# zc402/video-classification

Hardware: AMD Instinct MI355X
Metric: clips/sec SlowFast-R50 8x8, 32x224^2 bf16 training step (higher is better)
Workload: dtype bf16

## Files before the change

### video-classification_amd/csrc/conv_igemm.hip

```cpp

#include "conv_igemm_epi.h"

using namespace sfk_igemm;

namespace sfk_igemm {
__attribute__((visibility("hidden"))) int launch_p8(const ConvK& k, int bms, dim3 grid, hipStream_t s, int* dry);
__attribute__((visibility("hidden"))) bool halo_ok(const sfk_conv_desc* d);
__attribute__((visibility("hidden"))) int halo_mtiles(const sfk_conv_desc* d);
__attribute__((visibility("hidden"))) int launch_halo(const ConvK& k, const sfk_conv_desc* d, hipStream_t s, int* dry);
}

namespace {

template <typename T, int BM, int BN, int WM, int WN, bool SHORTK, int EPI = 0>
__global__ __launch_bounds__(256, (sizeof(T) == 2 ? 3 : 1)) void conv_igemm_kernel(const ConvK k) {
  using TL = Tile<T>;
  constexpr int VEC = TL::VEC, SEGS = TL::SEGS, ROWB = TL::ROWB;
  constexpr int FM = BM / WM / 16, FN = co_frags(BN, WN);
  constexpr int RPI = 256 / SEGS;
  constexpr int XL = BM / RPI;
  constexpr int WL = (BN + RPI - 1) / RPI;
  constexpr int BUF = (BM + BN) * ROWB;
  static_assert(WM * WN == 4 && BM % RPI == 0, "tile shape");
  __shared__ __attribute__((aligned(16))) char smem[2 * BUF];
  __shared__ sfk_tap s_taps[SFK_MAX_TAPS + 1];
  __shared__ int s_xdelta[SFK_MAX_TAPS + 1];
  __shared__ int s_woff[SFK_MAX_TAPS + 1];
  if (threadIdx.x <= SFK_MAX_TAPS) {
    sfk_tap t = k.taps[threadIdx.x < SFK_MAX_TAPS ? threadIdx.x : 0];
    if ((int)threadIdx.x >= k.ntaps) { t.dt = -128; t.dh = 0; t.dw = 0; t.widx = 0; }
    s_taps[threadIdx.x] = t;
    s_xdelta[threadIdx.x] = (((int)t.dt * k.xh + (int)t.dh) * k.xw + (int)t.dw) * k.xld * (int)sizeof(T);
    s_woff[threadIdx.x] = (int)t.widx * k.cin * (int)sizeof(T);
  }
  __syncthreads();

  const int tid = threadIdx.x, lane = tid & 63, wave = tid >> 6;
  const int wm = wave % WM, wn = wave / WM;
  const int l15 = lane & 15, g = lane >> 4;

  int mt, nt;
  {
    const int nblk = gridDim.x, b = blockIdx.x;
    const int q = nblk >> 3, r = nblk & 7, xcd = b & 7;
    const int logical = (xcd < r ? xcd * (q + 1) : r * (q + 1) + (xcd - r) * q) + (b >> 3);
    nt = logical % k.ntiles;
    mt = logical / k.ntiles;
  }

  const int seg = tid % SEGS, row0 = tid / SEGS;
  int xtb[XL], xhb[XL], xwb[XL];
  uint32_t xbase[XL];
#pragma unroll
  for (int i = 0; i < XL; ++i) {
    const int m = mt * BM + row0 + i * RPI;
    uint32_t q1, rw_, q2, rh_, n_, rt_;
    k.drw.divmod((uint32_t)m, q1, rw_);
    k.drh.divmod(q1, q2, rh_);
    k.drt.divmod(q2, n_, rt_);
    xtb[i] = (m < k.M) ? (int)rt_ * k.gst : -(1 << 28);
    xhb[i] = (int)rh_ * k.gsh;
    xwb[i] = (int)rw_ * k.gsw;
    xbase[i] = (uint32_t)((((((int64_t)n_ * k.xt + (int)rt_ * k.gst) * k.xh + xhb[i]) * k.xw + xwb[i]) * k.xld + k.xoff) *
                          (int64_t)sizeof(T));
  }
  uint32_t wbase[WL];
#pragma unroll
  for (int i = 0; i < WL; ++i) {
    const int r = row0 + i * RPI;
    const int co = nt * BN + r;
    wbase[i] = (r < BN && co < k.cout) ? (uint32_t)(co * k.wtaps * k.cin) * (uint32_t)sizeof(T) : SFK_OOB;
  }
  const __amdgpu_buffer_rsrc_t xrs = sfk_make_rsrc(k.x, k.xbytes);
  const __amdgpu_buffer_rsrc_t wrs = sfk_make_rsrc(k.w, k.wbytes);

  struct Stage { uint4 x[XL]; uint4 w[WL]; };
  auto gload = [&](int step, Stage& st) {
    const uint32_t q = (uint32_t)(step * SEGS + seg);
    uint32_t tap, cseg;
    k.dspt.divmod(q, tap, cseg);
    const bool cok = tap < (uint32_t)k.ntaps;
    const int ti_ = cok ? (int)tap : SFK_MAX_TAPS;
    const sfk_tap tp = s_taps[ti_];
    const uint32_t xd = (uint32_t)(s_xdelta[ti_] + (int)cseg * 16);
    const uint32_t wd = (uint32_t)(s_woff[ti_] + (int)cseg * 16);
#pragma unroll
    for (int i = 0; i < XL; ++i) {
      const int ti = xtb[i] + tp.dt, hi = xhb[i] + tp.dh, wi = xwb[i] + tp.dw;
      const bool ok = cok && (unsigned)ti < (unsigned)k.xt && (unsigned)hi < (unsigned)k.xh &&
                      (unsigned)wi < (unsigned)k.xw;
      st.x[i] = sfk_buffer_load16(xrs, ok ? xbase[i] + xd : SFK_OOB);
    }
#pragma unroll
    for (int i = 0; i < WL; ++i)
      st.w[i] = sfk_buffer_load16(wrs, (cok && wbase[i] != SFK_OOB) ? wbase[i] + wd : SFK_OOB);
  };
  auto lstore = [&](int buf, const Stage& st) {
    char* xs = smem + buf * BUF;
    char* ws = xs + BM * ROWB;
#pragma unroll
    for (int i = 0; i < XL; ++i) *reinterpret_cast<uint4*>(xs + TL::off(row0 + i * RPI, seg)) = st.x[i];
#pragma unroll
    for (int i = 0; i < WL; ++i) {
      const int r = row0 + i * RPI;
      if ((BN % RPI == 0) || r < BN) *reinterpret_cast<uint4*>(ws + TL::off(r, seg)) = st.w[i];
    }
  };

  f32x4 acc[FN][FM];
#pragma unroll
  for (int i = 0; i < FN; ++i)
#pragma unroll
    for (int j = 0; j < FM; ++j) acc[i][j] = f32x4{0.f, 0.f, 0.f, 0.f};

  auto compute = [&](int buf) {
    const char* xs = smem + buf * BUF;
    const char* ws = xs + BM * ROWB;
    typename TL::frag a[FN], b[FM];
#pragma unroll
    for (int i = 0; i < FN; ++i) a[i] = TL::load(ws, wn * (BN / WN) + 16 * i + l15, g);
#pragma unroll
    for (int j = 0; j < FM; ++j) b[j] = TL::load(xs, wm * (BM / WM) + 16 * j + l15, g);
#pragma unroll
    for (int i = 0; i < FN; ++i)
#pragma unroll
      for (int j = 0; j < FM; ++j) TL::mma(acc[i][j], a[i], b[j]);
  };

  Stage r0, r1;
  if constexpr (SHORTK) {
    gload(0, r0);
    lstore(0, r0);
    if (k.KC > 1) gload(1, r1);
    __syncthreads();
    int it = 0;
    for (; it + 3 < k.KC; it += 2) {
      gload(it + 2, r0);
      compute(0);
      lstore(1, r1);
      __syncthreads();
      gload(it + 3, r1);
      compute(1);
      lstore(0, r0);
      __syncthreads();
    }
    const int rem = k.KC - it;
    if (rem == 1) {
      compute(0);
    } else if (rem == 2) {
      compute(0);
      lstore(1, r1);
      __syncthreads();
      compute(1);
    } else {
      gload(it + 2, r0);
      compute(0);
      lstore(1, r1);
      __syncthreads();
      compute(1);
      lstore(0, r0);
      __syncthreads();
      compute(0);
    }
  } else {
    const int nit2 = (k.KC + 1) & ~1;
    gload(0, r0);
    lstore(0, r0);
    gload(1, r1);
    __syncthreads();
    for (int it = 0; it < nit2; it += 2) {
      gload(it + 2, r0);
      compute(0);
      lstore(1, r1);
      __syncthreads();
      gload(it + 3, r1);
      compute(1);
      lstore(0, r0);
      __syncthreads();
    }
  }

  if constexpr ((EPI == 1 || EPI >= 5) && sizeof(T) == 2 && (FN % 2) == 0) {
    __syncthreads();
    if constexpr (EPI == 5) epilogue_bits_sum<FM, FN, BM, BN, WM, WN>(k, acc, reinterpret_cast<float*>(smem), mt, nt, wm, wn, lane, tid);
    else epilogue_bn_bwd<FM, FN, BM, BN, WM, WN, EPI == 6, EPI == 7>(k, acc, reinterpret_cast<float*>(smem), mt, nt, wm, wn, lane, tid);
    return;
  }
  if constexpr (EPI == 3) {
    epilogue_fused<T, FM, FN, BM, BN, WM, WN>(k, acc, mt, nt, wm, wn, lane);
    return;
  }
  epilogue_plain<T, EPI, FM, FN, BM, BN, WM, WN, true>(k, acc, reinterpret_cast<float*>(smem), mt, nt, wm, wn, lane, tid);
}

typedef __attribute__((address_space(3))) void lds_void_t;

template <int BM, int BN, int WM, int WN, int EPI = 0, int BMS = BM>
__global__ __launch_bounds__(64 * WM * WN, (BN == 256 ? 2 : (WM * WN == 8 ? 4 : 3))) void conv_igemm_dma_kernel(const ConvK k) {
  using T = bf16_t;
  using TL = Tile<bf16_t>;
  constexpr int VEC = 8, SEGS = 4, ROWB = 64;
  constexpr int FM = BMS / WM / 16, FN = co_frags(BN, WN);
  static_assert(BMS <= BM && BMS % (16 * WM) == 0, "computed rows");
  constexpr int NW = WM * WN;
  constexpr int WROWS = BN < 16 * NW ? 16 * NW : BN;
  constexpr int XI = BM / (16 * NW), WI = WROWS / (16 * NW);
  constexpr int BUF = (BM + WROWS) * ROWB;
  constexpr int RED = WM * BN * 2 * 4;
  constexpr int SM = 3 * BUF > RED ? 3 * BUF : RED;
  constexpr int TAB = 32;
  static_assert((NW == 4 || NW == 8) && BM % (16 * NW) == 0, "tile shape");
  __shared__ __attribute__((aligned(16))) char smem[SM + 3 * TAB * 4];
  sfk_tap* s_taps = reinterpret_cast<sfk_tap*>(smem + SM);
  int* s_xdelta = reinterpret_cast<int*>(smem + SM) + TAB;
  int* s_woff = reinterpret_cast<int*>(smem + SM) + 2 * TAB;
  if (threadIdx.x <= SFK_MAX_TAPS) {
    sfk_tap t = k.taps[threadIdx.x < SFK_MAX_TAPS ? threadIdx.x : 0];
    if ((int)threadIdx.x >= k.ntaps) { t.dt = -128; t.dh = 0; t.dw = 0; t.widx = 0; }
    s_taps[threadIdx.x] = t;
    s_xdelta[threadIdx.x] = (((int)t.dt * k.xh + (int)t.dh) * k.xw + (int)t.dw) * k.xld * 2;
    s_woff[threadIdx.x] = (int)t.widx * k.cin * 2;
  }
  __syncthreads();

  const int tid = threadIdx.x, lane = tid & 63;
  const int wave = __builtin_amdgcn_readfirstlane(tid >> 6);
  const int wm = wave % WM, wn = wave / WM;
  const int l15 = lane & 15, g = lane >> 4;
  int mt, nt;
  {
    const int nblk = gridDim.x, b = blockIdx.x;
    const int q = nblk >> 3, r = nblk & 7, xcd = b & 7;
    const int logical = (xcd < r ? xcd * (q + 1) : r * (q + 1) + (xcd - r) * q) + (b >> 3);
    nt = logical % k.ntiles;
    mt = logical / k.ntiles;
  }

  const int lrow = lane >> 2;
  const int seg = (lane & 3) ^ ((4 - (((wave * (BM / NW) + lrow) >> 2) & 3)) & 3);
  static_assert((BM / NW) % 16 == 0 && (WROWS / NW) % 16 == 0, "row blocks");
  int xtb[XI], xhb[XI], xwb[XI];
  uint32_t xbase[XI];
#pragma unroll
  for (int j = 0; j < XI; ++j) {
    const int m = mt * BMS + wave * (BM / NW) + 16 * j + lrow;
    uint32_t q1, rw_, q2, rh_, n_, rt_;
    k.drw.divmod((uint32_t)m, q1, rw_);
    k.drh.divmod(q1, q2, rh_);
    k.drt.divmod(q2, n_, rt_);
    xtb[j] = (m < k.M) ? (int)rt_ * k.gst : -(1 << 28);
    xhb[j] = (int)rh_ * k.gsh;
    xwb[j] = (int)rw_ * k.gsw;
    xbase[j] = (uint32_t)((((((int64_t)n_ * k.xt + (int)rt_ * k.gst) * k.xh + xhb[j]) * k.xw + xwb[j]) * k.xld + k.xoff) * 2);
  }
  const int wseg = (lane & 3) ^ ((4 - (((wave * (WROWS / NW) + lrow) >> 2) & 3)) & 3);
  uint32_t wbase[WI];
#pragma unroll
  for (int j = 0; j < WI; ++j) {
    const int r = wave * (WROWS / NW) + 16 * j + lrow;
    const int co = nt * BN + r;
    wbase[j] = (r < BN && co < k.cout) ? (uint32_t)(co * k.wtaps * k.cin) * 2u : SFK_OOB;
  }
  const __amdgpu_buffer_rsrc_t xrs = sfk_make_rsrc(k.x, k.xbytes);
  const __amdgpu_buffer_rsrc_t wrs = sfk_make_rsrc(k.w, k.wbytes);

  const bool uniform = (k.cin & 31) == 0;
  const int kct = k.cin >> 5;
  constexpr uint32_t FAR = 0x80000000u;
  uint32_t xv[XI], wv[WI];

  auto issue = [&](int buf, const uint32_t (&xo)[XI], const uint32_t (&wo)[WI], int soff) __attribute__((always_inline)) {
    char* xs = smem + buf * BUF + wave * (BM / NW) * ROWB;
    char* ws = smem + buf * BUF + BM * ROWB + wave * (WROWS / NW) * ROWB;
#pragma unroll
    for (int j = 0; j < XI; ++j)
// ... 165 lines not shown
inline bool pw_plain_route(const sfk_conv_desc* d) {
  if (d->x.dtype != SFK_BF16 || !sfk_tune().igemm_pw_stream || (sfk_tune().igemm_pw_stream & 8) || d->stats || d->bnb.partials ||
      d->out_relu_bits || d->ep.res.ptr || d->ep.relu || d->ep.scale || !pointwise_lin(d) || (d->y.ld % 8) || (d->y.c_off % 8))
    return false;
  if (sfk_fmap_bytes(&d->y) >= (1ll << 32) - 64) return false;
  return (d->cout == 64 && d->cin == 64) || (d->cout == 128 && d->cin == 128) || (d->cout == 320 && d->cin == 128 && !d->accumulate && !d->ep.shift);
}
inline int pw_dgrad_rows(const sfk_conv_desc* d) {
  if (d->x.dtype != SFK_BF16 || !sfk_tune().igemm_pw_stream || (sfk_tune().igemm_pw_stream & 4) || !d->accumulate || ep_on(d) || d->stats || !d->out_relu_bits ||
      !d->bnb.partials || d->bnb.y_bn.ptr || !pointwise_lin(d) || !bnb_ok(d))
    return 0;
  return sfk_conv_pw_dgrad_rows(d);
}

int validate(const sfk_conv_desc* d) {
  if (!d || d->struct_size != sizeof(sfk_conv_desc)) return SFK_ERR_INVALID;
  if (!d->w) return SFK_ERR_INVALID;
  if (!sfk_fmap_ok(&d->x) || !sfk_fmap_ok(&d->y)) return SFK_ERR_INVALID;
  if (d->x.dtype != d->y.dtype || d->x.n != d->y.n) return SFK_ERR_INVALID;
  if (d->cin != d->x.c || d->cout != d->y.c) return SFK_ERR_INVALID;
  if (d->rt <= 0 || d->rh <= 0 || d->rw <= 0 || d->ntaps <= 0 || d->ntaps > SFK_MAX_TAPS) return SFK_ERR_INVALID;
  if (d->wtaps <= 0) return SFK_ERR_INVALID;
  for (int i = 0; i < d->ntaps; ++i)
    if (d->taps[i].widx >= d->wtaps) return SFK_ERR_INVALID;
  for (int a = 0; a < 3; ++a)
    if (d->gs[a] <= 0 || d->os[a] <= 0 || d->oo[a] < 0) return SFK_ERR_INVALID;
  if ((d->rt - 1) * d->os[0] + d->oo[0] >= d->y.t || (d->rh - 1) * d->os[1] + d->oo[1] >= d->y.h ||
      (d->rw - 1) * d->os[2] + d->oo[2] >= d->y.w)
    return SFK_ERR_INVALID;
  if ((int64_t)d->x.n * d->rt * d->rh * d->rw >= (1ll << 31)) return SFK_ERR_UNSUPPORTED;
  if (!sfk_fmap_vec_ok(&d->x)) return SFK_ERR_UNSUPPORTED;
  if ((d->y.c % 4) || (d->y.ld % 4) || (d->y.c_off % 4) || (((uintptr_t)d->y.ptr) & 15)) return SFK_ERR_UNSUPPORTED;
  if (((uintptr_t)d->w) & 15) return SFK_ERR_UNSUPPORTED;
  const bool bnb_bits = d->bnb.partials && !d->bnb.y_bn.ptr;
  if (d->out_relu_bits) {
    if (d->bnb.partials && !bnb_bits) return SFK_ERR_INVALID;
    if (!relu_out_ok(d)) return SFK_ERR_UNSUPPORTED;
  }
  if (ep_on(d)) {
    const sfk_conv_epilogue& e = d->ep;
    if (d->stats || d->bnb.partials || d->out_relu_bits) return SFK_ERR_INVALID;
    if ((e.relu_bits && !e.relu) || (e.res_scale && !e.res.ptr) || (e.res_shift && !e.res.ptr)) return SFK_ERR_INVALID;
    if (e.res.ptr && (!sfk_fmap_ok(&e.res) || e.res.n != d->y.n || e.res.t != d->y.t || e.res.h != d->y.h ||
                      e.res.w != d->y.w || e.res.c != d->y.c || e.res.dtype != d->y.dtype))
      return SFK_ERR_INVALID;
    if (!lin_out_of(d)) return SFK_ERR_UNSUPPORTED;
    if ((((uintptr_t)e.scale) | ((uintptr_t)e.shift) | ((uintptr_t)e.res_scale) | ((uintptr_t)e.res_shift)) & 15)
      return SFK_ERR_UNSUPPORTED;
    if (d->x.dtype == SFK_BF16) {
      if (d->cout > 16 ? !bnb_ok(d) : (e.res.ptr || e.relu)) return SFK_ERR_UNSUPPORTED;
    }
    if (e.res.ptr && !sfk_fmap_vec_ok(&e.res)) return SFK_ERR_UNSUPPORTED;
    if (sfk_fmap_bytes(&d->y) >= (1ll << 32) - 64 || (e.res.ptr && sfk_fmap_bytes(&e.res) >= (1ll << 32) - 64))
      return SFK_ERR_UNSUPPORTED;
  }
  if (d->bnb.partials) {
    if (sfk_fmap_bytes(&d->y) >= (1ll << 32) - 64) return SFK_ERR_UNSUPPORTED;
    if (d->bnb.y_bn.ptr && sfk_fmap_ok(&d->bnb.y_bn) && sfk_fmap_bytes(&d->bnb.y_bn) >= (1ll << 32) - 64) return SFK_ERR_UNSUPPORTED;
    if (d->bnb.mask_src.ptr && sfk_fmap_ok(&d->bnb.mask_src) && sfk_fmap_bytes(&d->bnb.mask_src) >= (1ll << 32) - 64) return SFK_ERR_UNSUPPORTED;
  }
  if (bnb_bits) {
    if (!d->out_relu_bits || d->stats || d->bnb.mask_src.ptr) return SFK_ERR_INVALID;
    if (!bnb_ok(d) || !lin_out_of(d)) return SFK_ERR_UNSUPPORTED;
  } else if (d->bnb.partials) {
    const sfk_bn_bwd_fuse& b = d->bnb;
    if (d->stats || !sfk_fmap_ok(&b.y_bn) || !b.mean || !b.invstd) return SFK_ERR_INVALID;
    if (b.y_bn.n != d->y.n || b.y_bn.t != d->y.t || b.y_bn.h != d->y.h || b.y_bn.w != d->y.w || b.y_bn.c != d->y.c ||
        b.y_bn.dtype != d->y.dtype)
      return SFK_ERR_INVALID;
    if (b.mask_src.ptr && (!sfk_fmap_ok(&b.mask_src) || b.mask_src.n != d->y.n || b.mask_src.t != d->y.t ||
                           b.mask_src.h != d->y.h || b.mask_src.w != d->y.w || b.mask_src.c != d->y.c ||
                           b.mask_src.dtype != d->y.dtype))
      return SFK_ERR_INVALID;
    if (!b.mask_src.ptr && b.relu && (!b.scale || !b.shift)) return SFK_ERR_INVALID;
    if (!bnb_ok(d)) return SFK_ERR_UNSUPPORTED;
    if (!sfk_fmap_vec_ok(&b.y_bn) || (b.mask_src.ptr && !sfk_fmap_vec_ok(&b.mask_src))) return SFK_ERR_UNSUPPORTED;
  }
  const int64_t esz = d->x.dtype == SFK_BF16 ? 2 : 4;
  if (sfk_fmap_bytes(&d->x) >= (1ll << 32) - 64 || (int64_t)d->cout * d->wtaps * d->cin * esz >= (1ll << 32) - 64)
    return SFK_ERR_UNSUPPORTED;
  return SFK_OK;
}

template <typename T, int BM, int BN, int WM, int WN, bool SHORTK, int EPI = 0>
int run_reg(const ConvK& k, dim3 grid, hipStream_t s, int* dry) {
  if (dry) {
    constexpr int FN = co_frags(BN, WN);
    const int wide = route_wide<T, FN, EPI>(k) ? 1 : 0;
    *dry = SFK_IGEMM_ROUTE(SFK_IK_REG, sizeof(T) == 2 ? 1 : 0, BM, BN, EPI, SHORTK ? 1 : 0, wide);
    return SFK_OK;
  }
  hipLaunchKernelGGL((conv_igemm_kernel<T, BM, BN, WM, WN, SHORTK, EPI>), grid, dim3(256), 0, s, k);
  SFK_CHECK_LAUNCH();
  return SFK_OK;
}
template <int BM, int BN, int WM, int WN, int EPI = 0, int BMS = BM>
int run_dma(const ConvK& k, dim3 grid, hipStream_t s, int* dry) {
  if (dry) {
    constexpr int FN = co_frags(BN, WN);
    const int wide = route_wide<bf16_t, FN, EPI>(k) ? 1 : 0;
    *dry = SFK_IGEMM_ROUTE(SFK_IK_DMA, 1, BMS, BN, EPI, 0, wide);
    return SFK_OK;
  }
  hipLaunchKernelGGL((conv_igemm_dma_kernel<BM, BN, WM, WN, EPI, BMS>), grid, dim3(64 * WM * WN), 0, s, k);
  SFK_CHECK_LAUNCH();
  return SFK_OK;
}

int launch_dma(const ConvK& k, int bm, dim3 grid, hipStream_t s, int bn, int* dry) {
  if (bn == 256) return bm == 224 ? run_dma<256, 256, 2, 4, 0, 224>(k, grid, s, dry) : run_dma<256, 256, 4, 2>(k, grid, s, dry);
  if (k.bn_parts) {
    if (k.bn_y == nullptr) return run_dma<128, 128, 2, 2, 5>(k, grid, s, dry);
    if (k.bn_mask) return run_dma<128, 128, 2, 2, 7>(k, grid, s, dry);
    if (k.accumulate) return run_dma<128, 128, 2, 2, 6>(k, grid, s, dry);
    return run_dma<128, 128, 2, 2, 1>(k, grid, s, dry);
  }
  if (k.ep_on) {
    if (bm == 256) return run_dma<256, 128, 4, 2, 3>(k, grid, s, dry);
    if (k.ep_res) return run_dma<128, 128, 2, 2, 4>(k, grid, s, dry);
    return run_dma<128, 128, 2, 2, 3>(k, grid, s, dry);
  }
  if (k.obits) return bm == 256 ? run_dma<256, 128, 4, 2, 2>(k, grid, s, dry) : run_dma<128, 128, 2, 2, 2>(k, grid, s, dry);
  return bm == 256 ? run_dma<256, 128, 4, 2>(k, grid, s, dry) : run_dma<128, 128, 2, 2>(k, grid, s, dry);
}

template <typename T>
int launch(const sfk_conv_desc* d, hipStream_t s, int* dry = nullptr) {
  ConvK k;
  k.x = d->x.ptr; k.y = d->y.ptr; k.w = d->w; k.stats = d->stats;
  k.xt = d->x.t; k.xh = d->x.h; k.xw = d->x.w; k.xld = d->x.ld; k.xoff = d->x.c_off;
  k.yt = d->y.t; k.yh = d->y.h; k.yw = d->y.w; k.yld = d->y.ld; k.yoff = d->y.c_off;
  k.M = d->x.n * d->rt * d->rh * d->rw;
  k.drw.set(d->rw); k.drh.set(d->rh); k.drt.set(d->rt);
  k.gst = d->gs[0]; k.gsh = d->gs[1]; k.gsw = d->gs[2];
  k.ost = d->os[0]; k.osh = d->os[1]; k.osw = d->os[2];
  k.oot = d->oo[0]; k.ooh = d->oo[1]; k.oow = d->oo[2];
  k.cin = d->cin; k.cout = d->cout; k.wtaps = d->wtaps; k.ntaps = d->ntaps;
  const int vec = sfk_vec_of(d->x.dtype), segs = BK / vec;
  k.dspt.set(d->cin / vec);
  k.dkct.set(d->cin / 32 > 0 ? d->cin / 32 : 1);
  k.dk64.set(d->ntaps);
  k.KC = (d->ntaps * (d->cin / vec) + segs - 1) / segs;
  k.accumulate = d->accumulate;
  k.obits = d->out_relu_bits;
  k.bn_parts = d->bnb.partials;
  k.bn_y = nullptr; k.bn_mask = nullptr;
  if (k.bn_parts) {
    k.bn_y = d->bnb.y_bn.ptr; k.bn_yld = d->bnb.y_bn.ld; k.bn_yoff = d->bnb.y_bn.c_off;
    k.bn_mask = d->bnb.mask_src.ptr; k.bn_mld = d->bnb.mask_src.ld; k.bn_moff = d->bnb.mask_src.c_off;
    k.bn_relu = d->bnb.relu;
    k.bn_mean = d->bnb.mean; k.bn_invstd = d->bnb.invstd; k.bn_scale = d->bnb.scale; k.bn_shift = d->bnb.shift;
  }
  k.ep_on = ep_on(d) ? 1 : 0;
  k.ep_scale = d->ep.scale; k.ep_shift = d->ep.shift; k.ep_rscale = d->ep.res_scale; k.ep_rshift = d->ep.res_shift;
  k.ep_res = d->ep.res.ptr; k.ep_rld = d->ep.res.ld; k.ep_roff = d->ep.res.c_off;
  k.ep_relu = d->ep.relu; k.ep_bits = d->ep.relu_bits;
  k.ybytes = (uint32_t)sfk_fmap_bytes(&d->y);
  k.ybig = sfk_fmap_bytes(&d->y) >= (1ll << 32) - 64 ? 1 : 0;
  k.ep_rbytes = d->ep.res.ptr ? (uint32_t)sfk_fmap_bytes(&d->ep.res) : 0u;
  k.bn_ybytes = (k.bn_parts && d->bnb.y_bn.ptr) ? (uint32_t)sfk_fmap_bytes(&d->bnb.y_bn) : 0u;
  k.bn_mbytes = (k.bn_parts && d->bnb.mask_src.ptr) ? (uint32_t)sfk_fmap_bytes(&d->bnb.mask_src) : 0u;
  k.obits_bytes = d->out_relu_bits ? (uint32_t)(sfk_fmap_pixels(&d->y) * (d->cout / sfk_vec_of(d->x.dtype))) : 0u;
  k.kshort = sfk_tune().igemm_short_k;
  k.lin_out = lin_out_of(d);
  const int wide_ok = sfk_tune().igemm_wide_store;
  k.wide_store = (wide_ok || k.obits) && (d->cout % 8) == 0 && (d->y.ld % 8) == 0 && (d->y.c_off % 8) == 0;
  k.xbytes = (uint32_t)sfk_fmap_bytes(&d->x);
  k.wbytes = (uint32_t)((int64_t)d->cout * d->wtaps * d->cin * (d->x.dtype == SFK_BF16 ? 2 : 4));
  for (int i = 0; i < SFK_MAX_TAPS; ++i) k.taps[i] = d->taps[i < d->ntaps ? i : 0];
  if constexpr (sizeof(T) == 2) {
    if (k.ep_on && (d->ep.res.ptr || d->ep.relu) && !d->accumulate && sfk_tune().igemm_pw_stream && d->ntaps == 1 &&
        d->taps[0].dt == 0 && d->taps[0].dh == 0 && d->taps[0].dw == 0 && d->gs[0] == 1 && d->gs[1] == 1 && d->gs[2] == 1 &&
        k.lin_out && d->x.t == d->y.t && d->x.h == d->y.h && d->x.w == d->y.w) {
      const int r = sfk_conv_pw_fused(d, s, dry, SFK_IK_PWF);
      if (r != SFK_ERR_UNSUPPORTED) return r;
    }
    if (pw_dgrad_rows(d) > 0) return sfk_conv_pw_dgrad(d, s, dry);
    if (pw_plain_route(d)) {
      const int r = sfk_conv_pw_fused(d, s, dry, SFK_IK_PWP);
      if (r != SFK_ERR_UNSUPPORTED) return r;
    }
  }
  if constexpr (sizeof(T) == 2) {
    if (halo_ok(d)) {
      k.mtiles = halo_mtiles(d);
      k.ntiles = 1;
      return launch_halo(k, d, s, dry);
    }
  }
  const TileSel ts = pick_tile(d);
  k.mtiles = (k.M + ts.bm - 1) / ts.bm;
  k.ntiles = (d->cout + ts.bn - 1) / ts.bn;
  const dim3 grid((unsigned)(k.mtiles * k.ntiles));
  if (ts.p8) return launch_p8(k, ts.bm, grid, s, dry);
  if (ts.dma) return launch_dma(k, ts.bm, grid, s, ts.bn, dry);
  if (k.bn_parts) {
    if constexpr (sizeof(T) == 2) {
      if (k.bn_y == nullptr) {
        if (ts.bn == 128) return run_reg<T, 128, 128, 2, 2, false, 5>(k, grid, s, dry);
        if (ts.bn == 64) return run_reg<T, 256, 64, 4, 1, false, 5>(k, grid, s, dry);
        return run_reg<T, 256, 32, 4, 1, false, 5>(k, grid, s, dry);
      }
      if (k.bn_mask) {
        if (ts.bn == 128) return run_reg<T, 128, 128, 2, 2, false, 7>(k, grid, s, dry);
        if (ts.bn == 64) return run_reg<T, 256, 64, 4, 1, false, 7>(k, grid, s, dry);
        return run_reg<T, 256, 32, 4, 1, false, 7>(k, grid, s, dry);
      }
      if (k.accumulate) {
        if (ts.bn == 128) return run_reg<T, 128, 128, 2, 2, false, 6>(k, grid, s, dry);
        if (ts.bn == 64) return run_reg<T, 256, 64, 4, 1, false, 6>(k, grid, s, dry);
        return run_reg<T, 256, 32, 4, 1, false, 6>(k, grid, s, dry);
      }
      if (ts.bn == 128) return run_reg<T, 128, 128, 2, 2, false, 1>(k, grid, s, dry);
      if (ts.bn == 64) return run_reg<T, 256, 64, 4, 1, false, 1>(k, grid, s, dry);
      return run_reg<T, 256, 32, 4, 1, false, 1>(k, grid, s, dry);
    }
    return SFK_ERR_UNSUPPORTED;
  }
  if (k.ep_on) {
    if (ts.bn == 128) return run_reg<T, 128, 128, 2, 2, false, 3>(k, grid, s, dry);
    if (ts.bn == 64) return run_reg<T, 256, 64, 4, 1, false, 3>(k, grid, s, dry);
    if (ts.bn == 32) return run_reg<T, 256, 32, 4, 1, false, 3>(k, grid, s, dry);
    return run_reg<T, 256, 16, 4, 1, false, 3>(k, grid, s, dry);
  }
  if (k.obits) {
    if (ts.bn == 128) return run_reg<T, 128, 128, 2, 2, false, 2>(k, grid, s, dry);
    if (ts.bn == 64) return run_reg<T, 256, 64, 4, 1, false, 2>(k, grid, s, dry);
    if (ts.bn == 32) return run_reg<T, 256, 32, 4, 1, false, 2>(k, grid, s, dry);
    if constexpr (sizeof(T) == 4) return run_reg<T, 256, 16, 4, 1, false, 2>(k, grid, s, dry);
    return SFK_ERR_UNSUPPORTED;
  }
  if (k.KC <= k.kshort && ts.bn <= 32) {
    if (ts.bn == 32) return run_reg<T, 256, 32, 4, 1, true>(k, grid, s, dry);
    return run_reg<T, 256, 16, 4, 1, true>(k, grid, s, dry);
  }
  if (ts.bn == 128) return run_reg<T, 128, 128, 2, 2, false>(k, grid, s, dry);
  if (ts.bn == 64) return run_reg<T, 256, 64, 4, 1, false>(k, grid, s, dry);
  if (ts.bn == 32) return run_reg<T, 256, 32, 4, 1, false>(k, grid, s, dry);
  return run_reg<T, 256, 16, 4, 1, false>(k, grid, s, dry);
}

int route_of(const sfk_conv_desc* d) {
  int route = -1;
  const int r = d->x.dtype == SFK_BF16 ? launch<bf16_t>(d, nullptr, &route) : launch<float>(d, nullptr, &route);
  return r != SFK_OK ? r : route;
}

}

extern "C" int sfk_conv_igemm_mtiles(const sfk_conv_desc* d) {
  const int st = validate(d);
  if (st != SFK_OK) return st;
  const int rows = pw_dgrad_rows(d);
  if (rows > 0) return rows;
  if (halo_ok(d)) return halo_mtiles(d);
  const int64_t M = (int64_t)d->x.n * d->rt * d->rh * d->rw;
  const int bm = pick_tile(d).bm;
  return (int)((M + bm - 1) / bm);
}

extern "C" int sfk_conv_relu_out_supported(const sfk_conv_desc* d) {
  if (!d || d->struct_size != sizeof(sfk_conv_desc)) return 0;
  sfk_conv_desc c = *d;
  c.out_relu_bits = nullptr;
  if (validate(&c) != SFK_OK) return 0;
  return relu_out_ok(d) ? 1 : 0;
}

extern "C" int sfk_conv_igemm_route(const sfk_conv_desc* d) {
  const int st = validate(d);
  return st != SFK_OK ? st : route_of(d);
}

extern "C" int sfk_conv_igemm_family(const sfk_conv_desc* d) {
  if (validate(d) != SFK_OK) return -1;
  const int r = route_of(d);
  if (r < 0) return -1;
  const int kern = SFK_IGEMM_ROUTE_KERNEL(r);
  return (kern == SFK_IK_PWP || kern == SFK_IK_PWF || kern == SFK_IK_PWD) ? 3 : kern;
}

extern "C" int sfk_conv_epilogue_supported(const sfk_conv_desc* d) {
  return (d && ep_on(d) && validate(d) == SFK_OK) ? 1 : 0;
}

extern "C" int sfk_conv_bnb_supported(const sfk_conv_desc* d) {
  if (!d || d->struct_size != sizeof(sfk_conv_desc)) return 0;
  sfk_conv_desc c = *d;
  c.bnb.partials = nullptr;
  if (validate(&c) != SFK_OK) return 0;
  return bnb_ok(d) ? 1 : 0;
}

extern "C" int sfk_conv_igemm(const sfk_conv_desc* d, sfk_stream_t stream) {
  const int st = validate(d);
  if (st != SFK_OK) return st;
  hipStream_t s = static_cast<hipStream_t>(stream);
  return d->x.dtype == SFK_BF16 ? launch<bf16_t>(d, s) : launch<float>(d, s);
}
```

### video-classification_amd/csrc/conv_igemm_epi.h

```cpp
#pragma once
#include "sfk_common.h"
#include <stdlib.h>

namespace sfk_igemm {


struct ConvK {
  const void* x;
  void* y;
  const void* w;
  float* stats;
  int xt, xh, xw, xld, xoff;
  int yt, yh, yw, yld, yoff;
  int M;
  FastDiv drw, drh, drt;
  int gst, gsh, gsw, ost, osh, osw, oot, ooh, oow;
  int cin, cout, wtaps, ntaps, KC, accumulate;
  int mtiles, ntiles;
  int wide_store;
  int kshort;
  int lin_out;
  const void* bn_y;
  const void* bn_mask;
  int bn_yld, bn_yoff, bn_mld, bn_moff, bn_relu;
// ... 453 lines not shown
            }
            o[e] = (bf16_t)f;
          }
          *reinterpret_cast<bf16x8*>(yp + rows[j] * k.yld + k.yoff + co) = o;
          if (k.ep_bits) k.ep_bits[rows[j] * (k.cout >> 3) + (co >> 3)] = (uint8_t)bits;
        }
      }
    }
  } else {
#pragma unroll
    for (int i = 0; i < FN; ++i) {
      const int co = co_w + 16 * i + 4 * g;
      const bool cok = co < k.cout;
      const int cc = cok ? co : 0;
      float sc[4], sh[4], rs[4], rh[4];
      {
        const uint32_t cb = (uint32_t)cc * 4u, nb = (uint32_t)k.cout * 4u;
        const bool has_sc = k.ep_scale != nullptr, has_rs = rp && k.ep_rscale;
        const uint4 a0 = sfk_buffer_load16(sfk_make_rsrc(k.ep_scale, has_sc ? nb : 0u), cb);
        const uint4 b0 = sfk_buffer_load16(sfk_make_rsrc(k.ep_shift, k.ep_shift ? nb : 0u), cb);
        const uint4 c0 = sfk_buffer_load16(sfk_make_rsrc(k.ep_rscale, has_rs ? nb : 0u), cb);
        const uint4 d0 = sfk_buffer_load16(sfk_make_rsrc(k.ep_rshift, (rp && k.ep_rshift) ? nb : 0u), cb);
        const uint32_t av[4] = {a0.x, a0.y, a0.z, a0.w}, bv[4] = {b0.x, b0.y, b0.z, b0.w};
        const uint32_t cv[4] = {c0.x, c0.y, c0.z, c0.w}, dv[4] = {d0.x, d0.y, d0.z, d0.w};
#pragma unroll
        for (int e = 0; e < 4; ++e) {
          sc[e] = has_sc ? __uint_as_float(av[e]) : 1.f;
          sh[e] = __uint_as_float(bv[e]);
          rs[e] = has_rs ? __uint_as_float(cv[e]) : 1.f;
          rh[e] = __uint_as_float(dv[e]);
        }
      }
      float oldv[FM][4], resv[FM][4];
      if constexpr (sizeof(T) == 2) {
        const __amdgpu_buffer_rsrc_t r_old = sfk_make_rsrc(k.y, k.accumulate ? k.ybytes : 0u);
#pragma unroll
        for (int j = 0; j < FM; ++j) {
          const auto o2 = __builtin_amdgcn_raw_buffer_load_b64(r_old, (int)((rows[j] * k.yld + k.yoff + cc) * 2), 0, 0);
          const bf16x4 ob = __builtin_bit_cast(bf16x4, o2);
#pragma unroll
          for (int e = 0; e < 4; ++e) {
            oldv[j][e] = (float)ob[e];
            resv[j][e] = 0.f;
          }
        }
      } else {
#pragma unroll
        for (int j = 0; j < FM; ++j) {
#pragma unroll
          for (int e = 0; e < 4; ++e) {
            oldv[j][e] = k.accumulate ? (float)yp[rows[j] * k.yld + k.yoff + cc + e] : 0.f;
            resv[j][e] = rp ? (float)rp[rows[j] * k.ep_rld + k.ep_roff + cc + e] : 0.f;
          }
        }
      }
#pragma unroll
      for (int j = 0; j < FM; ++j) {
        if (!rok[j] || !cok) continue;
        uint32_t bits = 0;
        float f[4];
#pragma unroll
        for (int e = 0; e < 4; ++e) {
          f[e] = acc[i][j][e] * sc[e] + sh[e] + oldv[j][e];
          if (rp) f[e] += resv[j][e] * rs[e] + rh[e];
          if (k.ep_relu) {
            bits |= (f[e] > 0.f ? 1u : 0u) << e;
            f[e] = f[e] > 0.f ? f[e] : 0.f;
          }
        }
        T* op = yp + rows[j] * k.yld + k.yoff + co;
        if constexpr (sizeof(T) == 4) {
          *reinterpret_cast<float4*>(op) = make_float4(f[0], f[1], f[2], f[3]);
          if (k.ep_bits) k.ep_bits[rows[j] * (k.cout >> 2) + (co >> 2)] = (uint8_t)bits;
        } else {
          bf16x4 o;
          o[0] = (bf16_t)f[0]; o[1] = (bf16_t)f[1]; o[2] = (bf16_t)f[2]; o[3] = (bf16_t)f[3];
          *reinterpret_cast<bf16x4*>(op) = o;
        }
      }
    }
  }
}

template <typename T, int EPI, int FM, int FN, int BM, int BN, int WM, int WN, bool RING_BUSY>
__device__ __forceinline__ void epilogue_plain(const ConvK& k, const f32x4 (&acc)[FN][FM], float* red, int mt, int nt,
                                               int wm, int wn, int lane, int tid) {
  const int l15 = lane & 15, g = lane >> 4;
  T* __restrict__ yp = static_cast<T*>(k.y);
  const int co_w = nt * BN + wn * (BN / WN);
  const bool wide = wide_store_taken<T, FN>(k);
  int64_t poffs[FM];
#pragma unroll
  for (int j = 0; j < FM; ++j) {
    const int m = mt * BM + wm * (BM / WM) + 16 * j + l15;
    if (k.lin_out) {
      poffs[j] = (int64_t)m * k.yld + k.yoff;
    } else {
      uint32_t q1, rw_, q2, rh_, n_, rt_;
      k.drw.divmod((uint32_t)m, q1, rw_);
      k.drh.divmod(q1, q2, rh_);
      k.drt.divmod(q2, n_, rt_);
      const int to = (int)rt_ * k.ost + k.oot, ho = (int)rh_ * k.osh + k.ooh, wo = (int)rw_ * k.osw + k.oow;
      poffs[j] = ((((int64_t)n_ * k.yt + to) * k.yh + ho) * k.yw + wo) * k.yld + k.yoff;
    }
  }
  bf16x8 oldv[FM][(FN + 1) / 2];
  if constexpr (sizeof(T) == 2) {
    if (wide && k.accumulate && k.ybig) {
#pragma unroll
      for (int j = 0; j < FM; ++j) {
        const int m = mt * BM + wm * (BM / WM) + 16 * j + l15;
        if (m < k.M) {
#pragma unroll
          for (int i = 0; i < FN; i += 2) oldv[j][i / 2] = load8_old(yp + poffs[j], co_w + 16 * i, k.cout, g);
        }
      }
    } else if (wide) {
      const __amdgpu_buffer_rsrc_t r_old = sfk_make_rsrc(k.y, k.accumulate ? k.ybytes : 0u);
      const int64_t plast = k.lin_out ? ((int64_t)(k.M - 1) * k.yld + k.yoff) : poffs[0];
#pragma unroll
      for (int j = 0; j < FM; ++j) {
        const int m = mt * BM + wm * (BM / WM) + 16 * j + l15;
        const int64_t po = (k.lin_out && m >= k.M) ? plast : poffs[j];
#pragma unroll
        for (int i = 0; i < FN; i += 2) {
          const int co = co_w + 16 * i + 16 * (g & 1) + 8 * (g >> 1);
          oldv[j][i / 2] = __builtin_bit_cast(bf16x8, sfk_buffer_load16(r_old, (uint32_t)((po + (co < k.cout ? co : 0)) * 2)));
        }
      }
    }
  }
  static_assert(EPI != 2 || FN <= 8, "one packed bitmap word per fragment row");
  uint32_t mb[EPI == 2 ? FM : 1];
  bool masked = false;
  if constexpr (EPI == 2) {
    masked = wide && k.obits;
    if (masked) {
      const bool word = (FN == 4 || FN == 2) && (k.cout % (FN * 16)) == 0;
      const int sh = 8 * (2 * (g & 1) + (g >> 1));
      if (word) {
        uint2 w[FM];
#pragma unroll
        for (int j = 0; j < FM; ++j) {
          const int m = mt * BM + wm * (BM / WM) + 16 * j + l15;
          const uint8_t* bp = k.obits + (int64_t)(m < k.M ? m : k.M - 1) * (k.cout >> 3) + (co_w >> 3);
          if constexpr (FN == 4) w[j] = *reinterpret_cast<const uint2*>(bp);
          else w[j] = make_uint2(*reinterpret_cast<const uint32_t*>(bp), 0u);
        }
#pragma unroll
        for (int j = 0; j < FM; ++j) mb[j] = ((w[j].x >> sh) & 255u) | (((w[j].y >> sh) & 255u) << 8);
      } else {
#pragma unroll
        for (int j = 0; j < FM; ++j) {
          const int m = mt * BM + wm * (BM / WM) + 16 * j + l15;
          mb[j] = 0;
          if (m < k.M) {
#pragma unroll
            for (int i = 0; i < FN; i += 2) {
              const int co = co_w + 16 * i + 16 * (g & 1) + 8 * (g >> 1);
              if (co < k.cout) mb[j] |= (uint32_t)k.obits[(int64_t)m * (k.cout >> 3) + (co >> 3)] << (8 * (i / 2));
            }
          }
        }
      }
    }
  }
#pragma unroll
  for (int j = 0; j < FM; ++j) {
    const int m = mt * BM + wm * (BM / WM) + 16 * j + l15;
    if (m < k.M) {
      const int64_t poff = poffs[j];
      if (wide) {
#pragma unroll
        for (int i = 0; i < FN; i += 2)
          store8_pair(yp + poff, co_w + 16 * i, k.cout, acc[i][j], acc[(i + 1) % FN][j], g, k.accumulate != 0, oldv[j][i / 2],
                      (EPI == 2 && masked) ? (int)((mb[EPI == 2 ? j : 0] >> (8 * (i / 2))) & 255u) : -1);
      } else {
#pragma unroll
        for (int i = 0; i < FN; ++i) {
          const int co = co_w + 16 * i + 4 * g;
          if (co < k.cout) {
            int mbits = -1;
            if constexpr (EPI == 2 && sizeof(T) == 4) {
              if (k.obits) mbits = k.obits[(int64_t)m * (k.cout >> 2) + (co >> 2)] & 15;
            }
            store4(yp + poff + co, acc[i][j], k.accumulate != 0, mbits);
          }
        }
      }
    }
  }

  if (k.stats) {
    if constexpr (RING_BUSY) __syncthreads();
#pragma unroll
    for (int i = 0; i < FN; ++i) {
#pragma unroll
      for (int r = 0; r < 4; ++r) {
        float s1 = 0.f, s2 = 0.f;
#pragma unroll
        for (int j = 0; j < FM; ++j) {
          const float v = acc[i][j][r];
          s1 += v;
          s2 += v * v;
        }
        s1 = row16_sum(s1);
        s2 = row16_sum(s2);
        if (l15 == 15) {
          const int col = wn * (BN / WN) + 16 * i + 4 * g + r;
          red[(wm * BN + col) * 2 + 0] = s1;
          red[(wm * BN + col) * 2 + 1] = s2;
        }
      }
    }
    __syncthreads();
    if (tid < BN) {
      const int co = nt * BN + tid;
      if (co < k.cout) {
        float s1 = 0.f, s2 = 0.f;
#pragma unroll
        for (int w_ = 0; w_ < WM; ++w_) {
          s1 += red[(w_ * BN + tid) * 2 + 0];
          s2 += red[(w_ * BN + tid) * 2 + 1];
        }
        float* o = k.stats + ((int64_t)mt * k.cout + co) * 2;
        o[0] = s1;
        o[1] = s2;
      }
    }
  }
}

}
```

Measured before the change: 1142.

## Add persistent short-K conv kernel with resident filters and cross-tile prefetch

Replaces the templated SHORTK path of the register igemm kernel with a dedicated persistent kernel for small-K, narrow-N convolutions. The kernel keeps the whole filter slice in LDS for every K-step, launches only as many blocks as fit resident on the CUs, walks M-tiles in an XCD-aware order, and issues the next tile's input gather from inside the epilogue through a new hook. The aim is to remove per-tile filter reloads and launch/tail overhead, and to hide global load latency behind the epilogue stores. In exchange it uses more LDS, adds register pressure from the multi-stage gather buffers, and queries the CU count on the host.

Result: no change. 1147, median of 6 (+0.5%).

```diff
diff --git a/video-classification_amd/csrc/conv_igemm.hip b/video-classification_amd/csrc/conv_igemm.hip
--- a/video-classification_amd/csrc/conv_igemm.hip
+++ b/video-classification_amd/csrc/conv_igemm.hip
@@ -12,7 +12,7 @@
 
 namespace {
 
-template <typename T, int BM, int BN, int WM, int WN, bool SHORTK, int EPI = 0>
+template <typename T, int BM, int BN, int WM, int WN, int EPI = 0>
 __global__ __launch_bounds__(256, (sizeof(T) == 2 ? 3 : 1)) void conv_igemm_kernel(const ConvK k) {
   using TL = Tile<T>;
   constexpr int VEC = TL::VEC, SEGS = TL::SEGS, ROWB = TL::ROWB;
@@ -128,41 +128,7 @@
   };
 
   Stage r0, r1;
-  if constexpr (SHORTK) {
-    gload(0, r0);
-    lstore(0, r0);
-    if (k.KC > 1) gload(1, r1);
-    __syncthreads();
-    int it = 0;
-    for (; it + 3 < k.KC; it += 2) {
-      gload(it + 2, r0);
-      compute(0);
-      lstore(1, r1);
-      __syncthreads();
-      gload(it + 3, r1);
-      compute(1);
-      lstore(0, r0);
-      __syncthreads();
-    }
-    const int rem = k.KC - it;
-    if (rem == 1) {
-      compute(0);
-    } else if (rem == 2) {
-      compute(0);
-      lstore(1, r1);
-      __syncthreads();
-      compute(1);
-    } else {
-      gload(it + 2, r0);
-      compute(0);
-      lstore(1, r1);
-      __syncthreads();
-      compute(1);
-      lstore(0, r0);
-      __syncthreads();
-      compute(0);
-    }
-  } else {
+  {
     const int nit2 = (k.KC + 1) & ~1;
     gload(0, r0);
     lstore(0, r0);
@@ -191,6 +157,154 @@
     return;
   }
   epilogue_plain<T, EPI, FM, FN, BM, BN, WM, WN, true>(k, acc, reinterpret_cast<float*>(smem), mt, nt, wm, wn, lane, tid);
+}
+
+constexpr int SHORTK_MAX = 5;
+
+template <typename T, int BN, int KC>
+__global__ __launch_bounds__(256, (sizeof(T) == 2 ? 3 : 1)) void conv_igemm_shortk_kernel(const ConvK k) {
+  using TL = Tile<T>;
+  constexpr int BM = 256, WM = 4, WN = 1;
+  constexpr int SEGS = TL::SEGS, ROWB = TL::ROWB;
+  constexpr int FM = BM / WM / 16, FN = co_frags(BN, WN);
+  constexpr int RPI = 256 / SEGS;
+  constexpr int XL = BM / RPI;
+  constexpr int XBUF = BM * ROWB, WBUF = BN * ROWB;
+  constexpr int OFF_W = 2 * XBUF, OFF_RED = OFF_W + KC * WBUF, OFF_TAB = OFF_RED + WM * BN * 2 * 4, TAB = 32;
+  static_assert(KC >= 1 && KC <= SHORTK_MAX && BN <= RPI, "one filter row per thread and K-step");
+  constexpr int NR = (sizeof(T) == 2 && BN == 32 && KC == 5) ? 3 : KC;
+  static_assert(SFK_MAX_TAPS + 1 <= TAB && sizeof(sfk_tap) == 4, "tap tables");
+  __shared__ __attribute__((aligned(16))) char smem[OFF_TAB + 3 * TAB * 4];
+  uint32_t* s_taps = reinterpret_cast<uint32_t*>(smem + OFF_TAB);
+  int* s_xdelta = reinterpret_cast<int*>(smem + OFF_TAB) + TAB;
+  int* s_woff = reinterpret_cast<int*>(smem + OFF_TAB) + 2 * TAB;
+  if (threadIdx.x <= SFK_MAX_TAPS) {
+    sfk_tap t = k.taps[threadIdx.x < SFK_MAX_TAPS ? threadIdx.x : 0];
+    if ((int)threadIdx.x >= k.ntaps) { t.dt = -128; t.dh = 0; t.dw = 0; t.widx = 0; }
+    s_taps[threadIdx.x] = (uint32_t)(uint8_t)t.dt | ((uint32_t)(uint8_t)t.dh << 8) | ((uint32_t)(uint8_t)t.dw << 16);
+    s_xdelta[threadIdx.x] = (((int)t.dt * k.xh + (int)t.dh) * k.xw + (int)t.dw) * k.xld * (int)sizeof(T);
+    s_woff[threadIdx.x] = (int)t.widx * k.cin * (int)sizeof(T);
+  }
+  __syncthreads();
+
+  const int tid = threadIdx.x, lane = tid & 63, wave = tid >> 6;
+  const int wm = wave;
+  const int l15 = lane & 15, g = lane >> 4;
+  const int seg = tid % SEGS, row0 = tid / SEGS;
+  const __amdgpu_buffer_rsrc_t xrs = sfk_make_rsrc(k.x, k.xbytes);
+  const __amdgpu_buffer_rsrc_t wrs = sfk_make_rsrc(k.w, k.wbytes);
+
+  uint32_t tpk[KC], xdl[KC];
+  {
+    uint4 wreg[KC];
+    const bool wrow = row0 < BN && row0 < k.cout;
+    const uint32_t wbase = (uint32_t)(row0 * k.wtaps * k.cin) * (uint32_t)sizeof(T);
+#pragma unroll
+    for (int s = 0; s < KC; ++s) {
+      uint32_t tap, cseg;
+      k.dspt.divmod((uint32_t)(s * SEGS + seg), tap, cseg);
+      const bool cok = tap < (uint32_t)k.ntaps;
+      const int ti_ = cok ? (int)tap : SFK_MAX_TAPS;
+      tpk[s] = s_taps[ti_] | (cok ? 1u << 24 : 0u);
+      xdl[s] = (uint32_t)(s_xdelta[ti_] + (int)cseg * 16);
+      wreg[s] = sfk_buffer_load16(wrs, (cok && wrow) ? wbase + (uint32_t)(s_woff[ti_] + (int)cseg * 16) : SFK_OOB);
+    }
+    if (row0 < BN) {
+#pragma unroll
+      for (int s = 0; s < KC; ++s) *reinterpret_cast<uint4*>(smem + OFF_W + s * WBUF + TL::off(row0, seg)) = wreg[s];
+    }
+  }
+
+  int xtb[XL], xhb[XL], xwb[XL];
+  uint32_t xbase[XL];
+  auto coords = [&](int mt, bool live) __attribute__((always_inline)) {
+#pragma unroll
+    for (int i = 0; i < XL; ++i) {
+      const int m = mt * BM + row0 + i * RPI;
+      uint32_t q1, rw_, q2, rh_, n_, rt_;
+      k.drw.divmod((uint32_t)m, q1, rw_);
+      k.drh.divmod(q1, q2, rh_);
+      k.drt.divmod(q2, n_, rt_);
+      xtb[i] = (live && m < k.M) ? (int)rt_ * k.gst : -(1 << 28);
+      xhb[i] = (int)rh_ * k.gsh;
+      xwb[i] = (int)rw_ * k.gsw;
+      xbase[i] = (uint32_t)((((((int64_t)n_ * k.xt + (int)rt_ * k.gst) * k.xh + xhb[i]) * k.xw + xwb[i]) * k.xld + k.xoff) *
+                            (int64_t)sizeof(T));
+    }
+  };
+  struct Stage { uint4 x[XL]; };
+  Stage st[NR];
+  auto gather_step = [&](int s) __attribute__((always_inline)) {
+    {
+      const int dt = (int)(int8_t)(tpk[s] & 255u), dh = (int)(int8_t)((tpk[s] >> 8) & 255u), dw = (int)(int8_t)((tpk[s] >> 16) & 255u);
+      const bool cok = (tpk[s] >> 24) != 0u;
+#pragma unroll
+      for (int i = 0; i < XL; ++i) {
+        const int ti = xtb[i] + dt, hi = xhb[i] + dh, wi = xwb[i] + dw;
+        const bool ok = cok && (unsigned)ti < (unsigned)k.xt && (unsigned)hi < (unsigned)k.xh && (unsigned)wi < (unsigned)k.xw;
+        st[s % NR].x[i] = sfk_buffer_load16(xrs, ok ? xbase[i] + xdl[s] : SFK_OOB);
+      }
+    }
+  };
+  auto gather = [&]() __attribute__((always_inline)) {
+#pragma unroll
+    for (int s = 0; s < NR; ++s) gather_step(s);
+  };
+  auto lstore = [&](int slot, const Stage& r) __attribute__((always_inline)) {
+#pragma unroll
+    for (int i = 0; i < XL; ++i) *reinterpret_cast<uint4*>(smem + slot * XBUF + TL::off(row0 + i * RPI, seg)) = r.x[i];
+  };
+
+  f32x4 acc[FN][FM];
+  auto compute = [&](int slot, int s) __attribute__((always_inline)) {
+    const char* xs = smem + slot * XBUF;
+    const char* ws = smem + OFF_W + s * WBUF;
+    typename TL::frag a[FN], b[FM];
+#pragma unroll
+    for (int i = 0; i < FN; ++i) a[i] = TL::load(ws, 16 * i + l15, g);
+#pragma unroll
+    for (int j = 0; j < FM; ++j) b[j] = TL::load(xs, wm * (BM / WM) + 16 * j + l15, g);
+#pragma unroll
+    for (int i = 0; i < FN; ++i)
+#pragma unroll
+      for (int j = 0; j < FM; ++j) TL::mma(acc[i][j], a[i], b[j]);
+  };
+
+  const int G = gridDim.x, ntile = k.mtiles;
+  const int tq = ntile >> 3, tr = ntile & 7;
+  auto tile_of = [&](int v) {
+    const int xcd = v & 7;
+    return (xcd < tr ? xcd * (tq + 1) : tr * (tq + 1) + (xcd - tr) * tq) + (v >> 3);
+  };
+  int v = blockIdx.x;
+  int mt = tile_of(v);
+  coords(mt, true);
+  gather();
+  for (;;) {
+#pragma unroll
+    for (int i = 0; i < FN; ++i)
+#pragma unroll
+      for (int j = 0; j < FM; ++j) acc[i][j] = f32x4{0.f, 0.f, 0.f, 0.f};
+#pragma unroll
+    for (int s = 0; s < KC; ++s) {
+      lstore(s & 1, st[s % NR]);
+      if (s + NR < KC) gather_step(s + NR);
+      __syncthreads();
+      compute(s & 1, s);
+    }
+    const int vn = v + G;
+    const bool more = vn < ntile;
+    const int mtn = more ? tile_of(vn) : mt;
+    epilogue_plain<T, 0, FM, FN, BM, BN, WM, WN, false>(k, acc, reinterpret_cast<float*>(smem + OFF_RED), mt, 0, wm, 0, lane, tid,
+                                                        [&]() __attribute__((always_inline)) {
+                                                          coords(mtn, more);
+                                                          gather();
+                                                        });
+    if (!more) break;
+    if constexpr (KC & 1) __syncthreads();
+    v = vn;
+    mt = mtn;
+  }
 }
 
 typedef __attribute__((address_space(3))) void lds_void_t;
@@ -522,15 +636,48 @@
   return SFK_OK;
 }
 
-template <typename T, int BM, int BN, int WM, int WN, bool SHORTK, int EPI = 0>
+template <typename T, int BM, int BN, int WM, int WN, int EPI = 0>
 int run_reg(const ConvK& k, dim3 grid, hipStream_t s, int* dry) {
   if (dry) {
     constexpr int FN = co_frags(BN, WN);
     const int wide = route_wide<T, FN, EPI>(k) ? 1 : 0;
-    *dry = SFK_IGEMM_ROUTE(SFK_IK_REG, sizeof(T) == 2 ? 1 : 0, BM, BN, EPI, SHORTK ? 1 : 0, wide);
+    *dry = SFK_IGEMM_ROUTE(SFK_IK_REG, sizeof(T) == 2 ? 1 : 0, BM, BN, EPI, 0, wide);
     return SFK_OK;
   }
-  hipLaunchKernelGGL((conv_igemm_kernel<T, BM, BN, WM, WN, SHORTK, EPI>), grid, dim3(256), 0, s, k);
+  hipLaunchKernelGGL((conv_igemm_kernel<T, BM, BN, WM, WN, EPI>), grid, dim3(256), 0, s, k);
+  SFK_CHECK_LAUNCH();
+  return SFK_OK;
+}
+
+inline int shortk_resident(int per_cu) {
+  static int cus = 0;
+  if (cus <= 0) {
+    int dev = 0, n = 0;
+    if (hipGetDevice(&dev) != hipSuccess || hipDeviceGetAttribute(&n, hipDeviceAttributeMultiprocessorCount, dev) != hipSuccess || n <= 0)
+      return -1;
+    cus = n;
+  }
+  return cus * per_cu;
+}
+template <typename T, int BN>
+int run_shortk(const ConvK& k, hipStream_t s, int* dry) {
+  if (dry) {
+    const int wide = route_wide<T, co_frags(BN, 1), 0>(k) ? 1 : 0;
+    *dry = SFK_IGEMM_ROUTE(SFK_IK_REG, sizeof(T) == 2 ? 1 : 0, 256, BN, 0, 1, wide);
+    return SFK_OK;
+  }
+  if (k.ntiles != 1) return SFK_ERR_UNSUPPORTED;
+  const int res = shortk_resident(sizeof(T) == 2 ? 3 : 1);
+  if (res <= 0) return SFK_ERR_LAUNCH;
+  const dim3 grid((unsigned)(k.mtiles < res ? k.mtiles : res));
+  switch (k.KC) {
+    case 1: hipLaunchKernelGGL((conv_igemm_shortk_kernel<T, BN, 1>), grid, dim3(256), 0, s, k); break;
+    case 2: hipLaunchKernelGGL((conv_igemm_shortk_kernel<T, BN, 2>), grid, dim3(256), 0, s, k); break;
+    case 3: hipLaunchKernelGGL((conv_igemm_shortk_kernel<T, BN, 3>), grid, dim3(256), 0, s, k); break;
+    case 4: hipLaunchKernelGGL((conv_igemm_shortk_kernel<T, BN, 4>), grid, dim3(256), 0, s, k); break;
+    case 5: hipLaunchKernelGGL((conv_igemm_shortk_kernel<T, BN, 5>), grid, dim3(256), 0, s, k); break;
+    default: return SFK_ERR_UNSUPPORTED;
+  }
   SFK_CHECK_LAUNCH();
   return SFK_OK;
 }
@@ -637,47 +784,47 @@
   if (k.bn_parts) {
     if constexpr (sizeof(T) == 2) {
       if (k.bn_y == nullptr) {
-        if (ts.bn == 128) return run_reg<T, 128, 128, 2, 2, false, 5>(k, grid, s, dry);
-        if (ts.bn == 64) return run_reg<T, 256, 64, 4, 1, false, 5>(k, grid, s, dry);
-        return run_reg<T, 256, 32, 4, 1, false, 5>(k, grid, s, dry);
+        if (ts.bn == 128) return run_reg<T, 128, 128, 2, 2, 5>(k, grid, s, dry);
+        if (ts.bn == 64) return run_reg<T, 256, 64, 4, 1, 5>(k, grid, s, dry);
+        return run_reg<T, 256, 32, 4, 1, 5>(k, grid, s, dry);
       }
       if (k.bn_mask) {
-        if (ts.bn == 128) return run_reg<T, 128, 128, 2, 2, false, 7>(k, grid, s, dry);
-        if (ts.bn == 64) return run_reg<T, 256, 64, 4, 1, false, 7>(k, grid, s, dry);
-        return run_reg<T, 256, 32, 4, 1, false, 7>(k, grid, s, dry);
+        if (ts.bn == 128) return run_reg<T, 128, 128, 2, 2, 7>(k, grid, s, dry);
+        if (ts.bn == 64) return run_reg<T, 256, 64, 4, 1, 7>(k, grid, s, dry);
+        return run_reg<T, 256, 32, 4, 1, 7>(k, grid, s, dry);
       }
       if (k.accumulate) {
-        if (ts.bn == 128) return run_reg<T, 128, 128, 2, 2, false, 6>(k, grid, s, dry);
-        if (ts.bn == 64) return run_reg<T, 256, 64, 4, 1, false, 6>(k, grid, s, dry);
-        return run_reg<T, 256, 32, 4, 1, false, 6>(k, grid, s, dry);
+        if (ts.bn == 128) return run_reg<T, 128, 128, 2, 2, 6>(k, grid, s, dry);
+        if (ts.bn == 64) return run_reg<T, 256, 64, 4, 1, 6>(k, grid, s, dry);
+        return run_reg<T, 256, 32, 4, 1, 6>(k, grid, s, dry);
       }
-      if (ts.bn == 128) return run_reg<T, 128, 128, 2, 2, false, 1>(k, grid, s, dry);
-      if (ts.bn == 64) return run_reg<T, 256, 64, 4, 1, false, 1>(k, grid, s, dry);
-      return run_reg<T, 256, 32, 4, 1, false, 1>(k, grid, s, dry);
+      if (ts.bn == 128) return run_reg<T, 128, 128, 2, 2, 1>(k, grid, s, dry);
+      if (ts.bn == 64) return run_reg<T, 256, 64, 4, 1, 1>(k, grid, s, dry);
+      return run_reg<T, 256, 32, 4, 1, 1>(k, grid, s, dry);
     }
     return SFK_ERR_UNSUPPORTED;
   }
   if (k.ep_on) {
-    if (ts.bn == 128) return run_reg<T, 128, 128, 2, 2, false, 3>(k, grid, s, dry);
-    if (ts.bn == 64) return run_reg<T, 256, 64, 4, 1, false, 3>(k, grid, s, dry);
-    if (ts.bn == 32) return run_reg<T, 256, 32, 4, 1, false, 3>(k, grid, s, dry);
-    return run_reg<T, 256, 16, 4, 1, false, 3>(k, grid, s, dry);
+    if (ts.bn == 128) return run_reg<T, 128, 128, 2, 2, 3>(k, grid, s, dry);
+    if (ts.bn == 64) return run_reg<T, 256, 64, 4, 1, 3>(k, grid, s, dry);
+    if (ts.bn == 32) return run_reg<T, 256, 32, 4, 1, 3>(k, grid, s, dry);
+    return run_reg<T, 256, 16, 4, 1, 3>(k, grid, s, dry);
   }
   if (k.obits) {
-    if (ts.bn == 128) return run_reg<T, 128, 128, 2, 2, false, 2>(k, grid, s, dry);
-    if (ts.bn == 64) return run_reg<T, 256, 64, 4, 1, false, 2>(k, grid, s, dry);
-    if (ts.bn == 32) return run_reg<T, 256, 32, 4, 1, false, 2>(k, grid, s, dry);
-    if constexpr (sizeof(T) == 4) return run_reg<T, 256, 16, 4, 1, false, 2>(k, grid, s, dry);
+    if (ts.bn == 128) return run_reg<T, 128, 128, 2, 2, 2>(k, grid, s, dry);
+    if (ts.bn == 64) return run_reg<T, 256, 64, 4, 1, 2>(k, grid, s, dry);
+    if (ts.bn == 32) return run_reg<T, 256, 32, 4, 1, 2>(k, grid, s, dry);
+    if constexpr (sizeof(T) == 4) return run_reg<T, 256, 16, 4, 1, 2>(k, grid, s, dry);
     return SFK_ERR_UNSUPPORTED;
   }
-  if (k.KC <= k.kshort && ts.bn <= 32) {
-    if (ts.bn == 32) return run_reg<T, 256, 32, 4, 1, true>(k, grid, s, dry);
-    return run_reg<T, 256, 16, 4, 1, true>(k, grid, s, dry);
-  }
-  if (ts.bn == 128) return run_reg<T, 128, 128, 2, 2, false>(k, grid, s, dry);
-  if (ts.bn == 64) return run_reg<T, 256, 64, 4, 1, false>(k, grid, s, dry);
-  if (ts.bn == 32) return run_reg<T, 256, 32, 4, 1, false>(k, grid, s, dry);
-  return run_reg<T, 256, 16, 4, 1, false>(k, grid, s, dry);
+  if (k.KC <= k.kshort && k.KC <= SHORTK_MAX && ts.bn <= 32) {
+    if (ts.bn == 32) return run_shortk<T, 32>(k, s, dry);
+    return run_shortk<T, 16>(k, s, dry);
+  }
+  if (ts.bn == 128) return run_reg<T, 128, 128, 2, 2>(k, grid, s, dry);
+  if (ts.bn == 64) return run_reg<T, 256, 64, 4, 1>(k, grid, s, dry);
+  if (ts.bn == 32) return run_reg<T, 256, 32, 4, 1>(k, grid, s, dry);
+  return run_reg<T, 256, 16, 4, 1>(k, grid, s, dry);
 }
 
 int route_of(const sfk_conv_desc* d) {
diff --git a/video-classification_amd/csrc/conv_igemm_epi.h b/video-classification_amd/csrc/conv_igemm_epi.h
--- a/video-classification_amd/csrc/conv_igemm_epi.h
+++ b/video-classification_amd/csrc/conv_igemm_epi.h
@@ -559,9 +559,10 @@
   }
 }
 
-template <typename T, int EPI, int FM, int FN, int BM, int BN, int WM, int WN, bool RING_BUSY>
+struct EpiNoHook { __device__ __forceinline__ void operator()() const {} };
+template <typename T, int EPI, int FM, int FN, int BM, int BN, int WM, int WN, bool RING_BUSY, typename Hook = EpiNoHook>
 __device__ __forceinline__ void epilogue_plain(const ConvK& k, const f32x4 (&acc)[FN][FM], float* red, int mt, int nt,
-                                               int wm, int wn, int lane, int tid) {
+                                               int wm, int wn, int lane, int tid, Hook&& loads_issued = Hook()) {
   const int l15 = lane & 15, g = lane >> 4;
   T* __restrict__ yp = static_cast<T*>(k.y);
   const int co_w = nt * BN + wn * (BN / WN);
@@ -642,6 +643,7 @@
       }
     }
   }
+  loads_issued();
 #pragma unroll
   for (int j = 0; j < FM; ++j) {
     const int m = mt * BM + wm * (BM / WM) + 16 * j + l15;
```
